# daeheepark/TrajSDE

Measured on AMD Instinct MI355X. Metric: scenes/sec (K=6, 20 SDE steps, ~256 agents) at 1/2/4/8 MI355X; minADE match, higher is better.
Workload: dtype f32 (fp16x3 split: 22-bit operands on v_mfma_f32_16x16x32_f16, f32 accumulate)

## Files before the change

### trajsde_amd/csrc/kernels.hpp

```cpp
#pragma once
#include <hip/hip_runtime.h>
#include <stdint.h>

#include "dropout.hpp"
#include "layouts.hpp"
#include "philox.hpp"

namespace tsde {

__global__ void k_aa_center(const float* img, const float* x, const float* x_fake, const float* rot, const uint8_t* bos,
                            const int32_t* orig, int N, int Nt, int H, float* center, float* cn, float* q);
template <bool X6>
__global__ void k_edge_kv(const float* img, const float* geom, const int32_t* dst, const float* q, int64_t E, float* logits, float* v,
                          int heads);
template <int THREADS>
__global__ void k_edge_kv2(const float* img, const float* geom, const int32_t* dst, const float* q, int64_t E, float* logits, float* v,
                           int heads);
constexpr int SEG_REC = 96;
constexpr int SEG_STREAMS_512 = 256 * 8 * 32;
struct AttnPlan {
  int C;
  int64_t nstreams;
  int64_t rec_slots(int64_t targets) const { return targets + nstreams + 1; }
};
// ... 93 lines not shown
    const float* _nf = nullptr;                                                                                     \
    if ((heads) == 4) {                                                                                             \
      if (_d) TS_LAUNCH_TAG("k_edge_attn_rows<4>", false, (k_global_attn<4, false, true, false>), grid, block, lds, st, img, segptr, _ns, emb, q, _nf, _nf, R, agg, stats, drop); \
      else TS_LAUNCH_TAG("k_edge_attn_rows<4>", false, (k_global_attn<4, false, false, false>), grid, block, lds, st, img, segptr, _ns, emb, q, _nf, _nf, R, agg, stats, drop); \
    } else {                                                                                                        \
      if (_d) TS_LAUNCH_TAG("k_edge_attn_rows<8>", false, (k_global_attn<8, false, true, false>), grid, block, lds, st, img, segptr, _ns, emb, q, _nf, _nf, R, agg, stats, drop); \
      else TS_LAUNCH_TAG("k_edge_attn_rows<8>", false, (k_global_attn<8, false, false, false>), grid, block, lds, st, img, segptr, _ns, emb, q, _nf, _nf, R, agg, stats, drop); \
    }                                                                                                               \
  } while (0)
__global__ void k_seg_merge(const int32_t* segptr, const float* rec, EdgeCount ec, int C, int64_t R, float* agg, float* stats, int heads,
                            const float* img, const float* q, int add_cv, int rec_layout);
template <bool DROP, bool SAVE, bool PP>
__global__ void k_edge_attn3(const float* img, const float* geom, const int32_t* dst, const float* q, EdgeCount ec, int C, float* rec, int heads,
                             const int32_t* segptr, DropArg drop, float* emb_out);
template <bool X6>
__global__ void k_edge_embed(const float* img, const float* geom, EdgeCount ec, float* emb_out, int st_bf16);
bool rel_embed_fused();
constexpr int edge_embed2_lds(int threads) { return (EdgeL6G::SIZE + (threads / 64) * ROWSTAGE) * 4; }
__global__ void k_edge_embed2(const float* img, const float* geom, EdgeCount ec, float* emb_out, int st_bf16);
template <bool X6>
__global__ void k_global_edge(const float* img, const float* rel, const int32_t* src, const int32_t* dst, const float* q,
                              const float* kn, const float* vn, int64_t E, float* logits, float* v);
template <int HEADS, bool ST_BF16, bool DROP, bool NODE>
__global__ void k_global_attn(const float* img, const int32_t* segptr, const int32_t* src, const float* rel, const float* q, const float* kn,
                              const float* vn, int64_t N, float* agg, float* stats, DropArg drop);
__global__ void k_seg_softmax_agg(const int32_t* segptr, const float* logits, const float* v, int64_t R, float* agg, int heads, DropArg drop);
template <bool X6>
__global__ void k_node_update(const float* img, const float* agg, const float* xn, const float* x, int64_t R, float* x1, float* xn2, DropArg drop,
                              SegMerge mg);
__global__ void k_ffn6(const float* img, const float* x1, const float* xn2, int64_t R, float* out, DropArg drop);
__global__ void k_ffn(const float* img, const float* x1, const float* xn2, int64_t R, float* out, DropArg drop, int out_bf16);
template <int NQ, bool SPLITKV = false>
__global__ void k_node_proj(const float* img, const float* x, int64_t R, float* xn_out, float* p0, float* p1, float* p2);
__global__ void k_mode_proj(const float* norm_g, const float* proj_g, const float* x, int64_t N, float* out);

__global__ void k_enc_sde_step(const float* img, const float* h_in, const float* hidden0, int Nt, float dt, float sq, float sn, float cs,
                               int idx, int noise_step0, NoiseArg na, const uint8_t* nus, const int32_t* eos, const int32_t* pick_slot, float* h_ode,
                               float* diff_pick);
__global__ void k_enc_gru_step(const float* img, const float* h_ode, const float* x_t, int Nt, int N, int t, int TT, int idx,
                               const uint8_t* pad, const int32_t* orig, const int32_t* eos, float* h_out, float* local_out,
                               float* latent_t);

constexpr int COOP_TMAX = 4;
constexpr int COOP_RS = 68;
constexpr int COOP_TILE = 16 * COOP_RS;
constexpr int COOP_BIAS_VECS = 21;
constexpr int coop_lds_floats(int tiles) {
  return tiles * (COOP_TILE + 5 * (TSDE_SPLIT_H3 ? 1024 : COOP_TILE)) + tiles * 64 + COOP_BIAS_VECS * 64 + 32 * 3 * 64;
}
struct StepTab {
  float dt[32], sq[32], sn[32], cs[32];
};
struct RecurTape {
  float *HIN, *H1, *H2, *G1, *G2, *GS, *HODE, *XS, *U1, *R1, *UU, *RR, *RH, *N1, *NW;
};
template <int TW, bool SAVE>
__global__ void k_enc_recur_coop(const float* sde_img, const float* gru_img, const float* coop6, const float* h0, const float* aa_out, int Nt, int N, int H,
                                 int TT, int tiles_per_wg, StepTab tab, int noise_step0, NoiseArg na, const uint8_t* nus, const uint8_t* pad,
                                 const int32_t* orig, const int32_t* eos, const int32_t* pick_slot, float* kept, float* diff_pick,
                                 float* latent_ys, int aa_bf16, RecurTape tp);
struct RecurBwdCoopArgs {
  const float *gru_t, *sde_t;
  int Nt, N, H, TT;
  NoiseArg na;
  const uint8_t *pad, *nus;
  const int32_t *orig, *eos;
// ... 43 lines not shown
```

### trajsde_amd/csrc/layouts.hpp

```cpp
#pragma once
#ifndef TSDE_SPLIT_H3
#define TSDE_SPLIT_H3 1
#endif

namespace tsde {

#define TS_FIELD(name, size, prev) name = prev##_END, name##_END = name + (size)

constexpr int MAT64 = 64 * 64;

struct AaCenterL {
  enum : int {
    S_END = 0,
    TS_FIELD(W0, 128, S), TS_FIELD(B0, 64, W0), TS_FIELD(G1, 64, B0), TS_FIELD(E1, 64, G1),
    TS_FIELD(W3, MAT64, E1), TS_FIELD(B3, 64, W3), TS_FIELD(G4, 64, B3), TS_FIELD(E4, 64, G4),
    TS_FIELD(W6, MAT64, E4), TS_FIELD(B6, 64, W6), TS_FIELD(G7, 64, B6), TS_FIELD(E7, 64, G7),
    TS_FIELD(BOS, 21 * 64, E7), TS_FIELD(N1G, 64, BOS), TS_FIELD(N1B, 64, N1G),
    TS_FIELD(WQ, MAT64, N1B), TS_FIELD(BQ, 64, WQ),
    SIZE = BQ_END
  };
};

struct EdgeL {
  enum : int {
// ... 79 lines not shown
  enum : int {
    S_END = 0,
    TS_FIELD(WIH, MAT64X6, S), TS_FIELD(BIH, 64, WIH), TS_FIELD(WHH, MAT64X6, BIH), TS_FIELD(BHH, 64, WHH),
    TS_FIELD(WSELF, MAT64X6, BHH), TS_FIELD(BSELF, 64, WSELF), TS_FIELD(WOUT, MAT64X6, BSELF), TS_FIELD(BOUT, 64, WOUT),
    TS_FIELD(N2G, 64, BOUT), TS_FIELD(N2B, 64, N2G),
    SIZE = N2B_END
  };
};
struct FfnL6 {
  enum : int {
    S_END = 0,
    TS_FIELD(W1, 2 * MAT64X6, S), TS_FIELD(B1, 128, W1), TS_FIELD(W2, 2 * MAT64X6, B1), TS_FIELD(B2, 64, W2),
    HALF = B2_END, SIZE = 2 * B2_END
  };
};
static_assert(UpdL6::SIZE * 4 <= 160 * 1024 && FfnL6::HALF * 4 <= 160 * 1024, "split-precision node images must fit LDS");

struct FfnL {
  enum : int {
    S_END = 0,
    TS_FIELD(W1, 4 * MAT64, S), TS_FIELD(B1, 256, W1), TS_FIELD(W2, 4 * MAT64, B1), TS_FIELD(B2, 64, W2),
    SIZE = B2_END
  };
};

template <int NQ>
struct NodeProjL {
  enum : int {
    S_END = 0,
    TS_FIELD(N1G, 64, S), TS_FIELD(N1B, 64, N1G), TS_FIELD(W, NQ * MAT64, N1B), TS_FIELD(B, NQ * 64, W),
    SIZE = B_END
  };
};

struct GEdgeL {
  enum : int { S_END = 0, TS_FIELD(WKV, 2 * MAT64, S), TS_FIELD(BKV, 128, WKV), SIZE = BKV_END };
};

struct DriftL {
  enum : int {
    S_END = 0,
    TS_FIELD(W0, MAT64, S), TS_FIELD(WS, 64, W0), TS_FIELD(WC, 64, WS), TS_FIELD(B0, 64, WC),
    TS_FIELD(W2, MAT64, B0), TS_FIELD(B2, 64, W2), TS_FIELD(W4, MAT64, B2), TS_FIELD(B4, 64, W4),
    SIZE = B4_END
  };
};
struct DiffL {
  enum : int {
    S_END = 0,
    TS_FIELD(W0, MAT64, S), TS_FIELD(WS, 64, W0), TS_FIELD(WC, 64, WS), TS_FIELD(B0, 64, WC),
    TS_FIELD(W2, MAT64, B0), TS_FIELD(B2, 64, W2), TS_FIELD(W4, 64, B2), TS_FIELD(B4, 4, W4),
    SIZE = B4_END
  };
};

struct DriftL6 {
  enum : int {
    S_END = 0,
    TS_FIELD(W0, MAT64X6, S), TS_FIELD(WS, 64, W0), TS_FIELD(WC, 64, WS), TS_FIELD(B0, 64, WC),
    TS_FIELD(W2, MAT64X6, B0), TS_FIELD(B2, 64, W2), TS_FIELD(W4, MAT64X6, B2), TS_FIELD(B4, 64, W4),
    SIZE = B4_END
  };
};
struct DiffL6 {
  enum : int {
    S_END = 0,
// ... 321 lines not shown
```

### trajsde_amd/csrc/stages.hip

```cpp
#include "common.hpp"
#include "kernels.hpp"
#include "layouts.hpp"

#include <algorithm>
#include <cstdlib>

namespace tsde {

static bool edge_x6() { static bool v = []() { const char* e = getenv("TRAJSDE_EDGE_FP32"); return !(e && atoi(e) != 0); }(); return v; }
static bool edge_pair() { static bool v = []() { const char* e = getenv("TRAJSDE_EDGE_PAIR"); return !(e && atoi(e) == 0); }(); return v; }
static int pair_threads() { static int t = []() { const char* e = getenv("TRAJSDE_PAIR_THREADS"); const int v = e ? atoi(e) : 768; return v == 512 ? 512 : 768; }(); return t; }
static bool attn_fused() { static bool v = []() { const char* e = getenv("TRAJSDE_ATTN_FUSED"); return !(e && atoi(e) == 0); }(); return v && edge_x6() && edge_pair() && TSDE_SPLIT_H3; }
static int fused_threads() {
  static const int t = [] { const char* e = getenv("TRAJSDE_FUSED_THREADS"); const int v = e ? atoi(e) : 512; return v == 256 ? 256 : 512; }();
  return t;
}
static bool merge_in_update() { static const bool v = []() { const char* e = getenv("TRAJSDE_MERGE_KERNEL"); return !(e && atoi(e) != 0); }(); return v; }
static bool edge_pipe() { static const bool v = []() { const char* e = getenv("TRAJSDE_EDGE_PIPE"); return e && atoi(e) == 1; }(); return v; }
static bool fused_one_tile() { static const bool v = []() { const char* e = getenv("TRAJSDE_FUSED_TILES"); return e && atoi(e) == 1; }(); return v; }
static bool edge_pingpong() { static const bool v = []() { const char* e = getenv("TRAJSDE_EDGE_PINGPONG"); return e && atoi(e) != 0; }(); return v; }
static bool edge_tile32() { static const bool v = []() { const char* e = getenv("TRAJSDE_EDGE_TILE"); return e && atoi(e) == 32; }(); return v && TSDE_SPLIT_H3; }
static bool global_fused_env() { static const bool v = []() { const char* e = getenv("TRAJSDE_GLOBAL_UNFUSED"); return !(e && atoi(e) != 0); }(); return v; }
static int fused_streams() { return 256 * 256; }
static AttnPlan fused_plan(int64_t E) { return attn_plan(E, fused_streams()); }
// ... 25 lines not shown
    hA = c.take<float>(int64_t(g->Nt) * 64); hB = c.take<float>(int64_t(g->Nt) * 64); lat = c.take<float>(N * 64);
    al_xn = c.take<float>(N * 64); al_q = c.take<float>(N * 64);
    al_logits = c.take<float>(fused ? 8 : int64_t(g->E_la) * 8 + 8); al_v = c.take<float>(fused ? 64 : int64_t(g->E_la) * 64 + 64);
    al_agg = c.take<float>(N * 64); al_x1 = c.take<float>(N * 64); al_xn2 = c.take<float>(N * 64);
    total = c.off + 256;
    ok = c.ok;
  }
};

struct AggWs {
  float *rel, *xn, *q, *kn, *vn, *logits, *v, *agg, *x1, *xn2, *xa, *xb;
  int64_t total;
  bool ok;
  AggWs(const trajsde_batch* b, const trajsde_graph* g, void* ws, int64_t bytes) {
    Carver c(ws, bytes);
    const int64_t N = b->N, E = g->E_g;
    rel = c.take<float>(E * 64 + 64);
    xn = c.take<float>(N * 64); q = c.take<float>(N * 64); kn = c.take<float>(N * 64); vn = c.take<float>(N * 64);
    logits = c.take<float>(E * 8 + 8); v = c.take<float>(E * 64 + 64);
    agg = c.take<float>(N * 64); x1 = c.take<float>(N * 64); xn2 = c.take<float>(N * 64); xa = c.take<float>(N * 64); xb = c.take<float>(N * 64);
    total = c.off + 256;
    ok = c.ok;
  }
};

static bool node_x6() {
  static bool v = []() {
    const char* e = getenv("TRAJSDE_NODE_FP32");
    return e ? atoi(e) == 0 : !TSDE_SPLIT_H3;
  }();
  return v;
}

struct NodeImgs {
  const float *upd, *ffn, *upd6, *ffn6;
};
static int update_ffn(const NodeImgs& im, const float* agg, const float* xn, const float* x, int64_t R, float* x1, float* xn2, float* out,
                      hipStream_t st, const DropArg& drop = no_drop(), bool out_bf16 = false, const SegMerge& mg = no_merge()) {
  const int64_t ntiles = (R + 15) / 16;
  TS_REQUIRE(!(out_bf16 && node_x6()), "bf16 state storage needs the one-pass FFN kernel (default fp16x3 build, TRAJSDE_NODE_FP32 unset)");
  if (node_x6()) {
    TS_LAUNCH(k_node_update<true>, tile_grid(ntiles, threads_node(), UpdL6::SIZE * 4), threads_node(), UpdL6::SIZE * 4, st, im.upd6, agg, xn, x,
              R, x1, xn2, drop, mg);
    TS_LAUNCH(k_ffn6, tile_grid(ntiles, threads_node(), FfnL6::HALF * 4), threads_node(), FfnL6::HALF * 4, st, im.ffn6, x1, xn2, R, out, drop);
  } else {
    TS_LAUNCH(k_node_update<false>, tile_grid(ntiles, threads_node(), UpdL::SIZE * 4), threads_node(), UpdL::SIZE * 4, st, im.upd, agg, xn, x, R,
              x1, xn2, drop, mg);
    TS_LAUNCH(k_ffn, tile_grid(ntiles, threads_node(), FfnL::SIZE * 4), threads_node(), FfnL::SIZE * 4, st, im.ffn, x1, xn2, R, out, drop, out_bf16 ? 1 : 0);
  }
  return TRAJSDE_OK;
}
static int attention_tail(const NodeImgs& im, const int32_t* segptr, const float* logits, const float* v, const float* xn, const float* x,
                          int64_t R, float* agg, float* x1, float* xn2, float* out, hipStream_t st, int heads = 8,
                          const DropArg& drop = no_drop()) {
  TS_LAUNCH(k_seg_softmax_agg, cdiv(R, 4), 256, 0, st, segptr, logits, v, R, agg, heads, drop);
  return update_ffn(im, agg, xn, x, R, x1, xn2, out, st, drop);
}

int fused_edge_attention(const char* tag, bool dominant, const float* img, const float* geom, const int32_t* dst, const float* q,
                         const EdgeCount& ec, const int32_t* segptr, int64_t R, float* rec, float* agg, int heads, hipStream_t st,
                         const DropArg& drop, float* emb_out, float* stats, SegMerge* defer) {
  const int64_t E = ec.E;
  const AttnPlan pl = fused_plan(E);
  TS_REQUIRE(E < (int64_t(1) << 28), "fused edge attention: an edge list of 2^28 or more entries exceeds its 32-bit byte offsets; split the batch");
  if (E > 0) {
    const int threads = fused_threads();
    const int64_t streams = ec.dev ? std::min<int64_t>(E, fused_streams()) : pl.nstreams;
    const int per_wg = (fused_one_tile() ? 1024 : threads) / 64 * (fused_one_tile() ? 16 : 32);
    const int grid = xcd_grid((streams + per_wg - 1) / per_wg);
    const int lds = (EdgeL6F::LDS_SIZE + 256 * 64) * 4;
    const bool d = drop.p > 0.f, sv = emb_out != nullptr;
#define TS_EA2H(N_, D_, S_, L_, H_) TS_LAUNCH_TAG(tag, dominant, (k_edge_attn2<N_, D_, S_, L_, H_>), grid, threads, lds, st, img, geom, dst, q, ec, pl.C, rec, heads, segptr, drop, emb_out)
#define TS_EA2L(N_, D_, S_, L_) do { if (heads == 8) TS_EA2H(N_, D_, S_, L_, true); else TS_EA2H(N_, D_, S_, L_, false); } while (0)
// ... 337 lines not shown
static int aggregator_forward_impl(const trajsde_batch* b, const trajsde_graph* g, const float* blob, int num_layers, int num_modes,
                                   int num_heads, const float* local_embed, void* ws, int64_t ws_bytes, float* global_embed,
                                   const trajsde_dropout* dropout, void* stream_, bool rel_ready);

int trajsde_aggregator_forward_heads(const trajsde_batch* b, const trajsde_graph* g, const float* blob, int num_layers, int num_modes,
                                     int num_heads, const float* local_embed, void* ws, int64_t ws_bytes, float* global_embed,
                                     const trajsde_dropout* dropout, void* stream_) {
  return aggregator_forward_impl(b, g, blob, num_layers, num_modes, num_heads, local_embed, ws, ws_bytes, global_embed, dropout, stream_, false);
}

int trajsde_aggregator_forward_prepared(const trajsde_batch* b, const trajsde_graph* g, const float* blob, int num_layers, int num_modes,
                                        int num_heads, const float* local_embed, void* ws, int64_t ws_bytes, float* global_embed,
                                        const trajsde_dropout* dropout, void* stream_) {
  return aggregator_forward_impl(b, g, blob, num_layers, num_modes, num_heads, local_embed, ws, ws_bytes, global_embed, dropout, stream_, true);
}

static int aggregator_forward_impl(const trajsde_batch* b, const trajsde_graph* g, const float* blob, int num_layers, int num_modes,
                                   int num_heads, const float* local_embed, void* ws, int64_t ws_bytes, float* global_embed,
                                   const trajsde_dropout* dropout, void* stream_, bool rel_ready) {
  TS_REQUIRE(b && g && blob && local_embed && ws && global_embed, "aggregator_forward: null pointer");
  TS_REQUIRE(!dropout || (dropout->p >= 0.f && dropout->p < 1.f), "aggregator_forward: dropout p must be in [0, 1)");
  TS_REQUIRE(num_heads == 8 || num_heads == 4, "aggregator_forward: num_heads must be 8 or 4");
  TS_REQUIRE(g->g_src && g->g_segptr, "aggregator_forward: graph not compacted (call trajsde_graph_compact)");
  TS_REQUIRE(num_layers >= 0 && num_modes > 0, "aggregator_forward: bad layer/mode count");
  AggWs w(b, g, ws, ws_bytes);
  if (!w.ok) return fail(TRAJSDE_ERR_WORKSPACE, "aggregator_forward: workspace too small");
  hipStream_t st = static_cast<hipStream_t>(stream_);
  const int64_t N = b->N, E = g->E_g, ntiles = (N + 15) / 16, etiles = (E + 15) / 16;
  const bool split = rel_split_possible() && num_heads == 8 && (!dropout || dropout->p == 0.f) && E > 0;
  if (!rel_ready || split != rel_split_possible())
    if (int rc = aggregator_rel_embed(b, g, blob, w, st, split)) return rc;
  const float* x = local_embed;
  float* bufs[2] = {w.xa, w.xb};
  for (int i = 0; i < num_layers; ++i) {
    const float* lb = blob + AggBlob::layer(i);
    if (split)
      TS_LAUNCH((k_node_proj<3, true>), tile_grid(ntiles, 512, NodeProjL<3>::SIZE * 4), 512, NodeProjL<3>::SIZE * 4, st, lb + AggLayerL::QKV, x, N,
                w.xn, w.q, w.kn, w.vn);
    else
      TS_LAUNCH(k_node_proj<3>, tile_grid(ntiles, 512, NodeProjL<3>::SIZE * 4), 512, NodeProjL<3>::SIZE * 4, st, lb + AggLayerL::QKV, x, N,
                w.xn, w.q, w.kn, w.vn);
    float* out = bufs[i & 1];
    const NodeImgs im{lb + AggLayerL::UPD, lb + AggLayerL::FFN, lb + AggLayerL::UPD6, lb + AggLayerL::FFN6};
    const bool fused = global_fused_env() || num_heads != 8;
    const DropArg drop = dropout ? make_drop(dropout->p, dropout->seed, 2 + i) : no_drop();
    TS_REQUIRE(fused || drop.p == 0.f, "aggregator_forward: dropout needs the fused global attention (unset TRAJSDE_GLOBAL_UNFUSED)");
    TS_REQUIRE(fused || !state_bf16(), "aggregator_forward: bf16 state storage needs the fused global attention");
    TS_REQUIRE(fused || g->exact, "aggregator_forward: a graph from trajsde_graph_prepare_async needs the fused global attention");
    if (fused) {
      TS_REQUIRE(N < (1 << 23), "aggregator_forward: node rows are addressed with 32-bit byte offsets (N < 2^23)");
      if (split && rel_split_scene_cache() && b->batch != nullptr && b->A > 0 && b->A + 2 <= E * 8 + 8) {
        int32_t* scene_ptr = reinterpret_cast<int32_t*>(w.logits);
        if (i == 0)
          if (int rc = launch_scene_ptr(b->batch, b->N, b->A, g->g_src, g->g_dst, g->g_segptr, E, scene_ptr, st)) return rc;
        if (int rc = launch_global_attn_sc(lb + AggLayerL::ATTN, g->g_segptr, g->g_src, w.rel, w.q, w.kn, w.vn, N, b->A, b->batch, scene_ptr, w.agg, st))
          return rc;
      } else if (split) {
        if (int rc = launch_global_attn_h3(lb + AggLayerL::ATTN, g->g_segptr, g->g_src, w.rel, w.q, w.kn, w.vn, N, w.agg, st)) return rc;
      } else if (num_heads == 8 && !state_bf16() && drop.p == 0.f && gattn_mm_enabled()) {
        if (int rc = launch_global_attn_mm(lb + AggLayerL::ATTN, g->g_segptr, g->g_src, w.rel, w.q, w.kn, w.vn, N, w.agg, st)) return rc;
      } else if (num_heads == 8 && !state_bf16() && gattn_f32mm_enabled() && E > 0) {
        if (int rc = launch_global_attn_mf(lb + AggLayerL::ATTN, g->g_segptr, g->g_src, w.rel, w.q, w.kn, w.vn, N, w.agg, nullptr, drop, st)) return rc;
      } else {
        TS_GLOBAL_ATTN(num_heads, state_bf16(), drop, xcd_grid(cdiv(N, 4)), 256, 0, st, lb + AggLayerL::ATTN, g->g_segptr, g->g_src, w.rel, w.q, w.kn, w.vn, N, w.agg, static_cast<float*>(nullptr));
      }
      if (int rc = update_ffn(im, w.agg, w.xn, x, N, w.x1, w.xn2, out, st, drop)) return rc;
      x = out;
      continue;
    }
    if (E > 0) {
      if (edge_x6())
        TS_LAUNCH(k_global_edge<true>, tile_grid(etiles, 512, GEdgeL6::SIZE * 4), 512, GEdgeL6::SIZE * 4, st,
                  lb + AggLayerL::EDGE6, w.rel, g->g_src, g->g_dst, w.q, w.kn, w.vn, E, w.logits, w.v);
      else
        TS_LAUNCH(k_global_edge<false>, tile_grid(etiles, 512, GEdgeL::SIZE * 4), 512, GEdgeL::SIZE * 4, st,
                  lb + AggLayerL::EDGE, w.rel, g->g_src, g->g_dst, w.q, w.kn, w.vn, E, w.logits, w.v);
    }
    if (int rc = attention_tail(im, g->g_segptr, w.logits, w.v, w.xn, x, N, w.agg, w.x1, w.xn2, out, st)) return rc;
    x = out;
  }
  const int lds = (128 + MAT64 + 64) * 4;
  dim3 grid(tile_grid(ntiles, 512, lds), num_modes);
  TS_LAUNCH(k_mode_proj, grid, 512, lds, st, blob + AggBlob::norm(num_layers), blob + AggBlob::proj(num_layers, 0), x, N, global_embed);
  return TRAJSDE_OK;
}

}
```

### trajsde_amd/csrc/prep.hip

```cpp

#include <algorithm>
#include <cmath>
#include <limits>
#include <atomic>
#include <cstdlib>
#include <cstring>

#include "common.hpp"
#include "philox.hpp"
#include "tile.hpp"

namespace tsde {

__global__ void k_rotate(const float* __restrict__ ang, int N, const float* __restrict__ y, int F,
                         float* __restrict__ rot, float* __restrict__ y_rot) {
  const int per = F > 0 && y != nullptr ? F : 1;
  const int64_t idx = int64_t(blockIdx.x) * blockDim.x + threadIdx.x;
  if (idx >= int64_t(N) * per) return;
  const int i = int(idx / per), t = int(idx - int64_t(i) * per);
  const float s = sinf(ang[i]), c = cosf(ang[i]);
  if (t == 0) {
    f4 r = {c, -s, s, c};
    *reinterpret_cast<f4*>(rot + 4 * i) = r;
  }
// ... 2 lines not shown
    y_rot[(int64_t(i) * F + t) * 2] = a * c + b * s;
    y_rot[(int64_t(i) * F + t) * 2 + 1] = b * c - a * s;
  }
}


constexpr int DONE_WAYS = 16;
__device__ __forceinline__ bool last_block_done(unsigned int* counters , unsigned int total) {
  __shared__ int s_last;
  asm volatile("s_waitcnt vmcnt(0)" ::: "memory");
  __syncthreads();
  if (threadIdx.x == 0) {
    const unsigned way = blockIdx.x % DONE_WAYS;
    const unsigned quota = total / DONE_WAYS + (way < total % DONE_WAYS ? 1u : 0u);
    int last = 0;
    if (__hip_atomic_fetch_add(&counters[way], 1u, __ATOMIC_RELAXED, __HIP_MEMORY_SCOPE_AGENT) + 1u == quota) {
      unsigned ways_used = total < unsigned(DONE_WAYS) ? total : unsigned(DONE_WAYS);
      last = __hip_atomic_fetch_add(&counters[DONE_WAYS], 1u, __ATOMIC_RELAXED, __HIP_MEMORY_SCOPE_AGENT) + 1u == ways_used;
    }
    s_last = last;
  }
  __syncthreads();
  return s_last != 0;
}
struct CoherentI32 {
  __amdgpu_buffer_rsrc_t rs;
  __device__ __forceinline__ explicit CoherentI32(const int32_t* base)
      : rs(__builtin_amdgcn_make_buffer_rsrc(const_cast<int32_t*>(base), 0, 0xFFFFFFFF, 0x00020000)) {}
  __device__ __forceinline__ int32_t operator[](int i) const { return __builtin_amdgcn_raw_buffer_load_b32(rs, i * 4, 0, 16 ); }
};
__device__ __forceinline__ void store_through(int32_t* p, int32_t v) { __hip_atomic_store(p, v, __ATOMIC_RELAXED, __HIP_MEMORY_SCOPE_AGENT); }

constexpr int EPT = 16;
__device__ __forceinline__ void degree_body(int blk, const int64_t* __restrict__ ei, int E, int32_t* __restrict__ deg) {
  int d[EPT];
#pragma unroll
  for (int u = 0; u < EPT; ++u) {
    const int e = (blk * EPT + u) * 256 + int(threadIdx.x);
    d[u] = e < E ? int(ei[int64_t(E) + e]) : -1;
  }
#pragma unroll
  for (int u = 0; u < EPT; ++u)
    if (d[u] >= 0) atomicAdd(&deg[d[u]], 1);
}
__device__ __forceinline__ void scatter_body(int blk, const int64_t* __restrict__ ei, int E, const int32_t* __restrict__ rowptr,
                                             int32_t* __restrict__ deg, int32_t* __restrict__ out) {
  int d[EPT], p[EPT], src[EPT];
#pragma unroll
  for (int u = 0; u < EPT; ++u) {
    const int e = (blk * EPT + u) * 256 + int(threadIdx.x);
    d[u] = e < E ? int(ei[int64_t(E) + e]) : -1;
    src[u] = e < E ? int32_t(ei[e]) : 0;
  }
#pragma unroll
  for (int u = 0; u < EPT; ++u) p[u] = d[u] >= 0 ? rowptr[d[u]] + atomicSub(&deg[d[u]], 1) - 1 : -1;
#pragma unroll
  for (int u = 0; u < EPT; ++u)
    if (p[u] >= 0) out[p[u]] = src[u];
}
__device__ __forceinline__ void scatter_lane_body(int blk, const int64_t* __restrict__ lai, int E, const int32_t* __restrict__ rowptr,
                                                  int32_t* __restrict__ deg, int64_t* __restrict__ out) {
  int d[EPT], p[EPT];
  int64_t key[EPT];
#pragma unroll
  for (int u = 0; u < EPT; ++u) {
    const int e = (blk * EPT + u) * 256 + int(threadIdx.x);
    d[u] = e < E ? int(lai[int64_t(E) + e]) : -1;
    key[u] = e < E ? ((lai[e] << 32) | int64_t(e)) : 0;
  }
#pragma unroll
  for (int u = 0; u < EPT; ++u) p[u] = d[u] >= 0 ? rowptr[d[u]] + atomicSub(&deg[d[u]], 1) - 1 : -1;
#pragma unroll
  for (int u = 0; u < EPT; ++u)
    if (p[u] >= 0) out[p[u]] = key[u];
}
__global__ __launch_bounds__(256) void k_scatter2(const int64_t* __restrict__ ei, int E, const int32_t* __restrict__ rowptr, int32_t* __restrict__ deg,
                                                  int32_t* __restrict__ csr_src, int nb_a, const int64_t* __restrict__ lai, int Ea,
                                                  const int32_t* __restrict__ la_rowptr, int32_t* __restrict__ la_deg, int64_t* __restrict__ la_pack) {
  const int blk = blockIdx.x;
  if (blk < nb_a) scatter_body(blk, ei, E, rowptr, deg, csr_src);
  else scatter_lane_body(blk - nb_a, lai, Ea, la_rowptr, la_deg, la_pack);
}
template <typename T, typename EMIT>
__device__ __forceinline__ void sort_long_rows(int vblk, int vgrid, const int32_t* __restrict__ rowptr, int n_rows, T* __restrict__ vals,
                                               T* buf , int32_t* __restrict__ low_out, int32_t* __restrict__ row_out,
                                               const EMIT& emit) {
  const T INF = sizeof(T) == 8 ? T(INT64_MAX) : T(INT32_MAX);
  for (int row = vblk; row < n_rows; row += vgrid) {
    const int beg = rowptr[row], n = rowptr[row + 1] - beg;
    if (n <= 256) continue;
    if (row_out != nullptr)
      for (int i = threadIdx.x; i < n; i += blockDim.x) row_out[beg + i] = row;
    int P = 2;
    while (P < n) P <<= 1;
    if (P <= 4096) {
      for (int i = threadIdx.x; i < P; i += blockDim.x) buf[i] = i < n ? vals[beg + i] : INF;
      __syncthreads();
      for (int k = 2; k <= P; k <<= 1)
        for (int j = k >> 1; j > 0; j >>= 1) {
          for (int i = threadIdx.x; i < P; i += blockDim.x) {
            const int l = i ^ j;
            if (l > i) {
              const T vi = buf[i], vl = buf[l];
              const bool up = (i & k) == 0;
              if ((vi > vl) == up) {
                buf[i] = vl;
                buf[l] = vi;
              }
            }
          }
          __syncthreads();
        }
      for (int i = threadIdx.x; i < n; i += blockDim.x) {
        vals[beg + i] = buf[i];
// ... 239 lines not shown
    }
    int32_t inc[2] = {sum[0], sum[1]};
#pragma unroll
    for (int d = 1; d < 64; d <<= 1) {
      const int32_t o0 = __shfl_up(inc[0], d), o1 = __shfl_up(inc[1], d);
      if (lane >= d) { inc[0] += o0; inc[1] += o1; }
    }
    if (lane == 63) { s_w[0][wv] = inc[0]; s_w[1][wv] = inc[1]; }
    __syncthreads();
#pragma unroll
    for (int a = 0; a < 2; ++a) {
      int32_t run = s_carry[a] + inc[a] - sum[a];
      for (int w = 0; w < wv; ++w) run += s_w[a][w];
      int32_t* out = a ? out1 : out0;
#pragma unroll
      for (int c = 0; c < PT; ++c) {
        const int i = base + PT * t + c;
        if (i < n) out[i] = run;
        run += v[a][c];
      }
    }
    __syncthreads();
    if (t < 2) s_carry[t] += s_w[t][0] + s_w[t][1] + s_w[t][2] + s_w[t][3];
    __syncthreads();
  }
}

struct FirstPassArgs {
  int N, A, H, TT, L, P, E, Ea, b0, b1, b2, b3, b4, b5, blocks;
  const int64_t *edge_index, *lane_actor_index, *agent_index, *batch, *source;
  const uint8_t *bos, *pad;
  const float *x, *pos, *lane_pos, *lane_pad;
  int32_t *deg, *la_deg, *rowptr, *la_rowptr, *orig, *eos, *pick_slot;
  uint8_t* nus;
  float *x_fake, *lane_feat;
  float2 *pos_t, *x_t;
  uint32_t* vmask;
  unsigned int* done;
  NoiseArg na;
};
__global__ __launch_bounds__(256) void k_prep_first(const FirstPassArgs a) {
  const int blk = blockIdx.x, i = threadIdx.x;
  if (blk < a.b0) degree_body(blk, a.edge_index, a.E, a.deg);
  else if (blk < a.b1) degree_body(blk - a.b0, a.lane_actor_index, a.Ea, a.la_deg);
  else if (blk < a.b2) ext_nodes_body((blk - a.b1) * 256 + i, a.N, a.A, a.H, a.agent_index, a.batch, a.source, a.bos, a.orig, a.nus, a.eos, a.pick_slot);
  else if (blk < a.b3) fake_x_body((blk - a.b2) * 256 + i, a.A, a.H, a.x, a.agent_index, a.na, a.x_fake);
  else if (blk < a.b4) valid_mask_body((blk - a.b3) * 256 + i, a.N, a.H, a.TT, a.pad, a.vmask);
  else if (blk < a.b5) time_major_body(blk - a.b4, a.N, a.H, a.TT, a.pos, a.x, a.pos_t, a.x_t);
  else lane_feat_body((blk - a.b5) * 256 + i, a.L, a.P, a.lane_pos, a.lane_pad, a.lane_feat);
  if (!last_block_done(a.done, unsigned(a.blocks))) return;
  block_scan_two(a.deg, a.rowptr, a.la_deg, a.la_rowptr, a.N + 1);
}

__global__ __launch_bounds__(256) void k_row_sort2(int N, int nb_a, int nb_l, const int32_t* __restrict__ rowptr, int32_t* __restrict__ csr_src,
                                                   int32_t* __restrict__ csr_dst, const uint32_t* __restrict__ vmask, int tref, int E,
                                                   uint8_t* __restrict__ flags_g, const int32_t* __restrict__ la_rowptr,
                                                   int64_t* __restrict__ la_pack, int32_t* __restrict__ la_eid, int32_t* __restrict__ la_actor,
                                                   const float* __restrict__ vec, float radius, int Ea, uint8_t* __restrict__ flags_la) {
  __shared__ int64_t buf[4096];
  const int blk = blockIdx.x;
  if (blk == 0 && threadIdx.x == 0) {
    flags_g[E] = 0;
    flags_la[Ea] = 0;
  }
  if (blk < nb_a) {
    if (E <= 0) return;
    auto emit = [&](int p, int32_t sender, int row) { flags_g[p] = uint8_t((vmask[sender] >> tref) & (vmask[row] >> tref) & 1u); };
    row_sort_part<int32_t>(blk, nb_a, rowptr, N, csr_src, nullptr, csr_dst, reinterpret_cast<int32_t*>(buf), emit);
  } else {
    if (Ea <= 0) return;
    auto emit = [&](int p, int64_t packed, int row) {
      (void)row;
      const int64_t e = packed & 0xFFFFFFFFll;
      flags_la[p] = uint8_t(sqrtf(norm2_sq(vec[2 * e], vec[2 * e + 1])) < radius);
    };
    row_sort_part<int64_t>(blk - nb_a, nb_l, la_rowptr, N, la_pack, la_eid, la_actor, buf, emit);
  }
// ... 447 lines not shown
  return w.total;
}

static int graph_prepare(const trajsde_batch* b, const float* rot, float radius, const trajsde_noise* fake_noise, void* ws,
                         int64_t ws_bytes, trajsde_graph* out, void* stream_, bool sync) {
  if (int rc = check_batch(b)) return rc;
  TS_REQUIRE(rot && ws && out, "graph_prepare: null pointer");
  PrepWs w(b, ws, ws_bytes);
  if (!w.ok) return fail(TRAJSDE_ERR_WORKSPACE, "graph_prepare: workspace too small");
  hipStream_t st = static_cast<hipStream_t>(stream_);
  const int N = b->N, A = b->A, E = b->E, H = b->H, TT = b->TT, Ea = b->E_al, Nt = N + A;
  NoiseArg na{0, nullptr, nullptr};
  if (fake_noise) { na.seed = fake_noise->seed; na.z = fake_noise->z; na.row_ids = fake_noise->row_ids; na.seed_dev = fake_noise->seed_dev; }

  TS_HIP(hipMemsetAsync(w.deg, 0, size_t(w.zeroed_bytes), st));
  const int tref = H - 1;
  {
    ProfScope ps("k_prep_first", st);
    FirstPassArgs fa;
    fa.N = N; fa.A = A; fa.H = H; fa.TT = TT; fa.L = b->L; fa.P = b->lane_pts; fa.E = E; fa.Ea = Ea;
    fa.b0 = cdiv(E, 256 * EPT);
    fa.b1 = fa.b0 + cdiv(Ea, 256 * EPT);
    fa.b2 = fa.b1 + cdiv(Nt, 256);
    fa.b3 = fa.b2 + (A > 0 ? cdiv(A * ((2 * H + 3) / 4), 256) : 0);
    fa.b4 = fa.b3 + cdiv(N, 256);
    fa.b5 = fa.b4 + cdiv(int64_t(N) * H, 1024);
    fa.blocks = fa.b5 + (b->L > 0 ? cdiv(b->L, 256) : 0);
    fa.edge_index = b->edge_index; fa.lane_actor_index = b->lane_actor_index; fa.agent_index = b->agent_index; fa.batch = b->batch;
    fa.source = b->source; fa.bos = b->bos_mask; fa.pad = b->padding_mask; fa.x = b->x; fa.pos = b->positions;
    fa.lane_pos = b->lane_positions; fa.lane_pad = b->lane_paddings;
    fa.deg = w.deg; fa.la_deg = w.la_deg; fa.rowptr = w.rowptr; fa.la_rowptr = w.la_rowptr; fa.orig = w.orig; fa.eos = w.eos;
    fa.pick_slot = w.pick_slot; fa.nus = w.nus; fa.x_fake = w.x_fake; fa.lane_feat = w.lane_feat; fa.pos_t = w.pos_t; fa.x_t = w.x_t;
    fa.vmask = w.vmask; fa.done = w.done + 0; fa.na = na;
    k_prep_first<<<fa.blocks, 256, 0, st>>>(fa);
  }
  if (E > 0 || Ea > 0) {
    ProfScope ps("k_scatter2", st);
    const int nb_a = cdiv(E, 256 * EPT);
    k_scatter2<<<nb_a + cdiv(Ea, 256 * EPT), 256, 0, st>>>(b->edge_index, E, w.rowptr, w.deg, w.csr_src, nb_a, b->lane_actor_index, Ea, w.la_rowptr,
                                                     w.la_deg, w.la_pack);
  }
  {
    ProfScope ps("k_row_sort2", st);
    const int per_list = cdiv(N, 4) < 8192 ? cdiv(N, 4) : 8192;
    k_row_sort2<<<2 * per_list, 256, 0, st>>>(N, per_list, per_list, w.rowptr, w.csr_src, w.csr_dst, w.vmask, tref, E, w.flags_g, w.la_rowptr,
                                              w.la_pack, w.la_eid, w.la_actor, b->lane_actor_vectors, radius, Ea, w.flags_la);
  }
  {
    ProfScope ps("k_aa_count", st);
    const AaArgs aa = aa_args(b, w, rot, radius);
    k_aa_count<<<int(w.aa_blocks), 256, 0, st>>>(aa);
  }
  {
    ProfScope ps("k_scan_multi", st);
    ScanMultiArgs sa;
    std::memset(&sa, 0, sizeof(sa));
    int64_t nmax = 0;
    auto add = [&](const void* in, int32_t* out_, int64_t n, int u8, int inst) {
      ScanJob& j = sa.j[sa.njobs++];
      j.in = in; j.out = out_; j.n = int(n); j.u8 = u8; j.st = w.scan_st + int64_t(inst) * SCAN_WORDS;
      nmax = std::max(nmax, n);
    };
    add(w.aa_segptr, w.aa_segptr, w.n_aa + 1, 0, 0);
    add(w.flags_g, w.cpos_g, int64_t(E) + 1, 1, 1);
    add(w.flags_la, w.cpos_la, int64_t(Ea) + 1, 1, 2);
    TS_REQUIRE(nmax <= int64_t(SCAN_MAX_BLOCKS) * 65536, "graph stage: more than 33 M elements in a prefix sum");
    const int64_t per = (nmax + int64_t(SCAN_MAX_BLOCKS) * 1024 - 1) / (int64_t(SCAN_MAX_BLOCKS) * 1024);
    const int PER = per <= 8 ? 8 : (per <= 16 ? 16 : (per <= 32 ? 32 : 64));
    for (int q = 0; q < sa.njobs; ++q) {
      sa.j[q].blocks = cdiv(sa.j[q].n, PER * 1024);
      sa.blocks += sa.j[q].blocks;
    }
    if (PER == 8) k_scan_multi<8><<<sa.blocks, 1024, 0, st>>>(sa);
// ... 85 lines not shown
```

Before: 16130.

## Fuse node update, FFN and next-layer QKV projection into one kernel

Adds k_node_block, which runs the gated node update, both FFN linears, and optionally the next layer's layernorm and QKV projection in a single launch. It stages the weight images in two phases, reusing the same LDS region. This removes intermediate x1/xn2 global round trips and one or two kernel launches per aggregator layer. In exchange, each block restages weights per round with extra barriers. By default it is only used when all tiles fit in one round, and it writes xn into the buffer that is also read as input.

Result: no change. 16200, median of 6 (+0.4%).

```diff
diff --git a/trajsde_amd/csrc/kernels.hpp b/trajsde_amd/csrc/kernels.hpp
--- a/trajsde_amd/csrc/kernels.hpp
+++ b/trajsde_amd/csrc/kernels.hpp
@@ -149,6 +149,9 @@
 __global__ void k_ffn(const float* img, const float* x1, const float* xn2, int64_t R, float* out, DropArg drop, int out_bf16);
 template <int NQ, bool SPLITKV = false>
 __global__ void k_node_proj(const float* img, const float* x, int64_t R, float* xn_out, float* p0, float* p1, float* p2);
+template <bool PROJ>
+__global__ void k_node_block(const float* upd, const float* ffn, const float* proj, const float* agg, const float* xn, const float* x,
+                             int64_t R, float* out, SegMerge mg, float* xn_next, float* p0, float* p1, float* p2);
 __global__ void k_mode_proj(const float* norm_g, const float* proj_g, const float* x, int64_t N, float* out);
 
 __global__ void k_enc_sde_step(const float* img, const float* h_in, const float* hidden0, int Nt, float dt, float sq, float sn, float cs,
diff --git a/trajsde_amd/csrc/layouts.hpp b/trajsde_amd/csrc/layouts.hpp
--- a/trajsde_amd/csrc/layouts.hpp
+++ b/trajsde_amd/csrc/layouts.hpp
@@ -135,6 +135,16 @@
     SIZE = B_END
   };
 };
+
+struct NodeBlockL {
+  enum : int {
+    S_END = 0,
+    TS_FIELD(A, UpdL::SIZE, S), TS_FIELD(B, 4 * MAT64 + 256, A), TS_FIELD(B2, 64, B),
+    SIZE = B2_END
+  };
+};
+static_assert(FfnL::B1 == FfnL::W1 + 4 * MAT64 && 4 * MAT64 <= UpdL::SIZE && NodeProjL<3>::SIZE <= 4 * MAT64 + 256 &&
+              NodeBlockL::SIZE * 4 <= 160 * 1024, "k_node_block: the second images are staged over the first");
 
 struct GEdgeL {
   enum : int { S_END = 0, TS_FIELD(WKV, 2 * MAT64, S), TS_FIELD(BKV, 128, WKV), SIZE = BKV_END };
diff --git a/trajsde_amd/csrc/node_block.hip b/trajsde_amd/csrc/node_block.hip
--- /dev/null
+++ b/trajsde_amd/csrc/node_block.hip
@@ -0,0 +1,147 @@
+#include "common.hpp"
+#include "kernels.hpp"
+#include "layouts.hpp"
+#include "range.hpp"
+#include "tile.hpp"
+
+namespace tsde {
+
+#if TSDE_SPLIT_H3
+template <bool PROJ>
+__global__ __launch_bounds__(512) void k_node_block(const float* __restrict__ upd_g, const float* __restrict__ ffn_g,
+                                                    const float* __restrict__ proj_g, const float* __restrict__ agg, const float* xn,
+                                                    const float* __restrict__ x, int64_t R, float* __restrict__ out, SegMerge mg,
+                                                    float* xn_next, float* __restrict__ p0, float* __restrict__ p1,
+                                                    float* __restrict__ p2) {
+  extern __shared__ __attribute__((aligned(16))) float lds[];
+  using U = UpdL;
+  using P = NodeProjL<3>;
+  float* const lds_a = lds + NodeBlockL::A;
+  float* const lds_b = lds + NodeBlockL::B;
+  const float* const b2 = lds + NodeBlockL::B2;
+  const Lane L;
+  const int waves = blockDim.x >> 6, wave = __builtin_amdgcn_readfirstlane(int(threadIdx.x >> 6));
+  const int64_t ntiles = (R + 15) / 16;
+  stage_copy(lds + NodeBlockL::B2, ffn_g + FfnL::B2, 64);
+  const int64_t first = int64_t(blockIdx.x) * waves, stride = int64_t(gridDim.x) * waves;
+  for (int64_t base = first; base < ntiles; base += stride) {
+    if (base != first) __syncthreads();
+    stage_copy(lds_a, upd_g, U::SIZE);
+    stage_copy(lds_b, ffn_g + FfnL::W1, NodeBlockL::B_END - NodeBlockL::B);
+    __syncthreads();
+    keep_lds_reads_here();
+    const int64_t tile = base + wave;
+    const bool live = tile < ntiles;
+    const int64_t row = tile * 16 + L.n, r = row < R ? row : R - 1;
+    f4 x1[4], hid[16];
+    if (live) {
+      f4 a[4], n[4], g[4], s[4];
+      if (mg.rec != nullptr) {
+        const int C = stream_len(mg.ec, edge_count(mg.ec), mg.C_host);
+        const int beg = mg.segptr[r], end = mg.segptr[r + 1];
+#pragma unroll
+        for (int jt = 0; jt < 4; ++jt) a[jt] = f4{0.f, 0.f, 0.f, 0.f};
+        if (end > beg) {
+          const StreamMap smap = stream_map(C);
+          const int c0 = int(stream_of(smap, beg)), c1 = int(stream_of(smap, end - 1));
+          const float* rr = mg.rec + (r + c0) * SEG_REC;
+#pragma unroll
+          for (int jt = 0; jt < 4; ++jt) a[jt] = *reinterpret_cast<const f4*>(rr + 16 * jt + 4 * L.g);
+          f4 m = *reinterpret_cast<const f4*>(rr + 64 + 4 * L.g), sm = *reinterpret_cast<const f4*>(rr + 80 + 4 * L.g);
+          for (int c = c0 + 1; c <= c1; ++c) {
+            rr += SEG_REC;
+            const f4 mp = *reinterpret_cast<const f4*>(rr + 64 + 4 * L.g), sp = *reinterpret_cast<const f4*>(rr + 80 + 4 * L.g);
+#pragma unroll
+            for (int jt = 0; jt < 4; ++jt) {
+              const f4 ap = *reinterpret_cast<const f4*>(rr + 16 * jt + 4 * L.g);
+              const float mn = fmaxf(m[jt], mp[jt]);
+              const float wa = fast_exp(m[jt] - mn), wb = fast_exp(mp[jt] - mn);
+              sm[jt] = sm[jt] * wa + sp[jt] * wb;
+              a[jt] = a[jt] * wa + ap * wb;
+              m[jt] = mn;
+            }
+          }
+#pragma unroll
+          for (int jt = 0; jt < 4; ++jt) {
+            const f4 cv = *reinterpret_cast<const f4*>(mg.cv + 16 * jt + 4 * L.g);
+#pragma unroll
+            for (int c = 0; c < 4; ++c) a[jt][c] = a[jt][c] / (sm[jt] + 1e-16f) + cv[c];
+          }
+        }
+      } else {
+        load_row(a, agg, r, L.g);
+      }
+      load_row(n, xn, r, L.g);
+      f4 xr[4];
+      load_row(xr, x, r, L.g);
+      range_note(absmax<4>(a), RS_NODE_AGG);
+      linear<4, 4>(g, a, lds_a + U::WIH, lds_a + U::BIH, L);
+      {
+        f4 h[4];
+        linear<4, 4>(h, n, lds_a + U::WHH, lds_a + U::BHH, L);
+#pragma unroll
+        for (int jt = 0; jt < 4; ++jt) g[jt] += h[jt];
+      }
+      sigmoid_<4>(g);
+      linear<4, 4>(s, n, lds_a + U::WSELF, lds_a + U::BSELF, L);
+#pragma unroll
+      for (int jt = 0; jt < 4; ++jt)
+#pragma unroll
+        for (int c = 0; c < 4; ++c) a[jt][c] = a[jt][c] + g[jt][c] * (s[jt][c] - a[jt][c]);
+      range_note(absmax<4>(a), RS_NODE_AGG);
+      linear<4, 4>(s, a, lds_a + U::WOUT, lds_a + U::BOUT, L);
+#pragma unroll
+      for (int jt = 0; jt < 4; ++jt) x1[jt] = n[jt] = xr[jt] + s[jt];
+      layer_norm<4>(n, lds_a + U::N2G, lds_a + U::N2B, L.g);
+      linear<16, 4>(hid, n, lds_b, lds_b + 4 * MAT64, L);
+      relu<16>(hid);
+      range_note(absmax<16>(hid), RS_FFN_HIDDEN);
+    }
+    __syncthreads();
+    stage_copy(lds_a, ffn_g + FfnL::W2, 4 * MAT64);
+    if (PROJ) stage_copy(lds_b, proj_g, P::SIZE);
+    __syncthreads();
+    keep_lds_reads_here();
+    if (live) {
+      f4 o[4];
+      linear<4, 16>(o, hid, lds_a, b2, L);
+#pragma unroll
+      for (int jt = 0; jt < 4; ++jt) o[jt] += x1[jt];
+      if (row < R) store_row(o, out, row, L.g);
+      if (PROJ) {
+        f4 pr[12];
+        layer_norm<4>(o, lds_b + P::N1G, lds_b + P::N1B, L.g);
+        if (row < R) store_row(o, xn_next, row, L.g);
+        linear<12, 4>(pr, o, lds_b + P::W, lds_b + P::B, L);
+        float* outs[3] = {p0, p1, p2};
+#pragma unroll
+        for (int j = 0; j < 3; ++j) {
+          f4 t4[4] = {pr[4 * j], pr[4 * j + 1], pr[4 * j + 2], pr[4 * j + 3]};
+          if (j > 0) {
+            if (row < R) {
+              char* o8 = reinterpret_cast<char*>(outs[j] + row * 64);
+#pragma unroll
+              for (int jt = 0; jt < 4; ++jt) {
+                unsigned h0, l0, h1, l1;
+                split_pair(t4[jt][0], t4[jt][1], h0, l0);
+                split_pair(t4[jt][2], t4[jt][3], h1, l1);
+                *reinterpret_cast<uint2*>(o8 + 32 * jt + 8 * L.g) = uint2{h0, h1};
+                *reinterpret_cast<uint2*>(o8 + 128 + 32 * jt + 8 * L.g) = uint2{l0, l1};
+              }
+            }
+            continue;
+          }
+          if (row < R) store_row(t4, outs[j], row, L.g);
+        }
+      }
+    }
+  }
+}
+
+template __global__ void k_node_block<false>(const float*, const float*, const float*, const float*, const float*, const float*, int64_t, float*,
+                                             SegMerge, float*, float*, float*, float*);
+template __global__ void k_node_block<true>(const float*, const float*, const float*, const float*, const float*, const float*, int64_t, float*,
+                                            SegMerge, float*, float*, float*, float*);
+#endif
+
+}
diff --git a/trajsde_amd/csrc/stages.hip b/trajsde_amd/csrc/stages.hip
--- a/trajsde_amd/csrc/stages.hip
+++ b/trajsde_amd/csrc/stages.hip
@@ -81,13 +81,43 @@
   return v;
 }
 
+static int node_fuse() { static const int v = []() { const char* e = getenv("TRAJSDE_NODE_FUSE"); return e ? atoi(e) : 1; }(); return v; }
+constexpr int64_t NODE_BLOCK_ONE_ROUND = 256 * 8;
+static bool node_block_serves(int64_t R, const DropArg& drop, bool out_bf16) {
+#if TSDE_SPLIT_H3
+  static const bool plain = getenv("TRAJSDE_NODE_FP32") == nullptr && threads_node() == 512;
+  return plain && node_fuse() != 0 && drop.p == 0.f && !out_bf16 && R > 0 && (node_fuse() == 2 || (R + 15) / 16 <= NODE_BLOCK_ONE_ROUND);
+#else
+  (void)R; (void)drop; (void)out_bf16;
+  return false;
+#endif
+}
+
 struct NodeImgs {
   const float *upd, *ffn, *upd6, *ffn6;
 };
+struct NextProj {
+  const float* img;
+  float *xn, *q, *kn, *vn;
+};
 static int update_ffn(const NodeImgs& im, const float* agg, const float* xn, const float* x, int64_t R, float* x1, float* xn2, float* out,
-                      hipStream_t st, const DropArg& drop = no_drop(), bool out_bf16 = false, const SegMerge& mg = no_merge()) {
+                      hipStream_t st, const DropArg& drop = no_drop(), bool out_bf16 = false, const SegMerge& mg = no_merge(),
+                      const NextProj* next = nullptr) {
   const int64_t ntiles = (R + 15) / 16;
   TS_REQUIRE(!(out_bf16 && node_x6()), "bf16 state storage needs the one-pass FFN kernel (default fp16x3 build, TRAJSDE_NODE_FP32 unset)");
+#if TSDE_SPLIT_H3
+  if (node_block_serves(R, drop, out_bf16)) {
+    const int grid = tile_grid(ntiles, 512, NodeBlockL::SIZE * 4);
+    if (next)
+      TS_LAUNCH((k_node_block<true>), grid, 512, NodeBlockL::SIZE * 4, st, im.upd, im.ffn, next->img, agg, xn, x, R, out, mg, next->xn, next->q,
+                next->kn, next->vn);
+    else
+      TS_LAUNCH((k_node_block<false>), grid, 512, NodeBlockL::SIZE * 4, st, im.upd, im.ffn, static_cast<const float*>(nullptr), agg, xn, x, R, out,
+                mg, static_cast<float*>(nullptr), static_cast<float*>(nullptr), static_cast<float*>(nullptr), static_cast<float*>(nullptr));
+    return TRAJSDE_OK;
+  }
+#endif
+  TS_REQUIRE(next == nullptr, "update_ffn: the next layer's projection rides on the fused launch only");
   if (node_x6()) {
     TS_LAUNCH(k_node_update<true>, tile_grid(ntiles, threads_node(), UpdL6::SIZE * 4), threads_node(), UpdL6::SIZE * 4, st, im.upd6, agg, xn, x,
               R, x1, xn2, drop, mg);
@@ -491,9 +521,12 @@
     if (int rc = aggregator_rel_embed(b, g, blob, w, st, split)) return rc;
   const float* x = local_embed;
   float* bufs[2] = {w.xa, w.xb};
+  bool proj_done = false;
   for (int i = 0; i < num_layers; ++i) {
     const float* lb = blob + AggBlob::layer(i);
-    if (split)
+    if (proj_done)
+      proj_done = false;
+    else if (split)
       TS_LAUNCH((k_node_proj<3, true>), tile_grid(ntiles, 512, NodeProjL<3>::SIZE * 4), 512, NodeProjL<3>::SIZE * 4, st, lb + AggLayerL::QKV, x, N,
                 w.xn, w.q, w.kn, w.vn);
     else
@@ -523,7 +556,9 @@
       } else {
         TS_GLOBAL_ATTN(num_heads, state_bf16(), drop, xcd_grid(cdiv(N, 4)), 256, 0, st, lb + AggLayerL::ATTN, g->g_segptr, g->g_src, w.rel, w.q, w.kn, w.vn, N, w.agg, static_cast<float*>(nullptr));
       }
-      if (int rc = update_ffn(im, w.agg, w.xn, x, N, w.x1, w.xn2, out, st, drop)) return rc;
+      const NextProj next{blob + AggBlob::layer(i + 1) + AggLayerL::QKV, w.xn, w.q, w.kn, w.vn};
+      proj_done = split && i + 1 < num_layers && node_block_serves(N, drop, false);
+      if (int rc = update_ffn(im, w.agg, w.xn, x, N, w.x1, w.xn2, out, st, drop, false, no_merge(), proj_done ? &next : nullptr)) return rc;
       x = out;
       continue;
     }
```

## Rank edges per block in shared-memory hash table to cut global atomics in CSR build

Applied to the files above, without the earlier changes.

The degree-counting pass now groups each block's edges by destination in a shared-memory open-addressing hash table. It issues one global atomicAdd per distinct destination instead of one per edge, and records each edge's position within its row. The scatter pass reads these precomputed in-row positions instead of doing a global atomicSub per edge. This trades contended global atomics for shared-memory CAS work, an extra int32 write and read per edge, and LDS use in every k_prep_first block. It falls back to per-edge atomics when probing overflows, and it reuses the cpos_g/cpos_la buffers as scratch, which assumes those are free and large enough at this stage.

After: 16270 before, 16250 after, median of 2. No clear change (-0.1%).

```diff
diff --git a/trajsde_amd/csrc/prep.hip b/trajsde_amd/csrc/prep.hip
--- a/trajsde_amd/csrc/prep.hip
+++ b/trajsde_amd/csrc/prep.hip
@@ -58,34 +58,94 @@
 __device__ __forceinline__ void store_through(int32_t* p, int32_t v) { __hip_atomic_store(p, v, __ATOMIC_RELAXED, __HIP_MEMORY_SCOPE_AGENT); }
 
 constexpr int EPT = 16;
-__device__ __forceinline__ void degree_body(int blk, const int64_t* __restrict__ ei, int E, int32_t* __restrict__ deg) {
-  int d[EPT];
+constexpr int RANK_SLOTS = 1024, RANK_PROBES = 8;
+struct RankTable {
+  int32_t key[RANK_SLOTS];
+  int32_t cnt[RANK_SLOTS];
+  int overflow;
+};
+__device__ __forceinline__ bool block_rank(const int (&d)[EPT], int (&slot)[EPT], int (&r)[EPT], RankTable& s) {
+  const int tid = int(threadIdx.x);
+  for (int i = tid; i < RANK_SLOTS; i += 256) {
+    s.key[i] = -1;
+    s.cnt[i] = 0;
+  }
+  if (tid == 0) s.overflow = 0;
+  __syncthreads();
 #pragma unroll
   for (int u = 0; u < EPT; ++u) {
-    const int e = (blk * EPT + u) * 256 + int(threadIdx.x);
+    slot[u] = -1;
+    r[u] = 0;
+    if (d[u] < 0) continue;
+    int h = d[u] & (RANK_SLOTS - 1);
+    for (int probe = 0; probe < RANK_PROBES; ++probe) {
+      const int k = atomicCAS(&s.key[h], -1, d[u]);
+      if (k == -1 || k == d[u]) {
+        slot[u] = h;
+        break;
+      }
+      h = (h + 1) & (RANK_SLOTS - 1);
+    }
+    if (slot[u] >= 0) r[u] = atomicAdd(&s.cnt[slot[u]], 1);
+    else s.overflow = 1;
+  }
+  __syncthreads();
+  return s.overflow == 0;
+}
+__device__ __forceinline__ void degree_body(int blk, const int64_t* __restrict__ ei, int E, int32_t* __restrict__ deg,
+                                            int32_t* __restrict__ inrow, RankTable& s) {
+  const int tid = int(threadIdx.x);
+  int d[EPT], slot[EPT], r[EPT];
+#pragma unroll
+  for (int u = 0; u < EPT; ++u) {
+    const int e = (blk * EPT + u) * 256 + tid;
     d[u] = e < E ? int(ei[int64_t(E) + e]) : -1;
   }
+  if (!block_rank(d, slot, r, s)) {
+#pragma unroll
+    for (int u = 0; u < EPT; ++u) r[u] = d[u] >= 0 ? atomicAdd(&deg[d[u]], 1) : 0;
+#pragma unroll
+    for (int u = 0; u < EPT; ++u)
+      if (d[u] >= 0) inrow[(blk * EPT + u) * 256 + tid] = r[u];
+    return;
+  }
+  {
+    constexpr int SPT = RANK_SLOTS / 256;
+    int c[SPT], k[SPT];
+#pragma unroll
+    for (int q = 0; q < SPT; ++q) {
+      c[q] = s.cnt[q * 256 + tid];
+      k[q] = s.key[q * 256 + tid];
+    }
+#pragma unroll
+    for (int q = 0; q < SPT; ++q)
+      if (c[q] > 0) c[q] = atomicAdd(&deg[k[q]], c[q]);
+#pragma unroll
+    for (int q = 0; q < SPT; ++q) s.cnt[q * 256 + tid] = c[q];
+  }
+  __syncthreads();
 #pragma unroll
   for (int u = 0; u < EPT; ++u)
-    if (d[u] >= 0) atomicAdd(&deg[d[u]], 1);
+    if (d[u] >= 0) inrow[(blk * EPT + u) * 256 + tid] = s.cnt[slot[u]] + r[u];
 }
 __device__ __forceinline__ void scatter_body(int blk, const int64_t* __restrict__ ei, int E, const int32_t* __restrict__ rowptr,
-                                             int32_t* __restrict__ deg, int32_t* __restrict__ out) {
+                                             const int32_t* __restrict__ inrow, int32_t* __restrict__ out) {
   int d[EPT], p[EPT], src[EPT];
 #pragma unroll
   for (int u = 0; u < EPT; ++u) {
     const int e = (blk * EPT + u) * 256 + int(threadIdx.x);
     d[u] = e < E ? int(ei[int64_t(E) + e]) : -1;
     src[u] = e < E ? int32_t(ei[e]) : 0;
-  }
-#pragma unroll
-  for (int u = 0; u < EPT; ++u) p[u] = d[u] >= 0 ? rowptr[d[u]] + atomicSub(&deg[d[u]], 1) - 1 : -1;
+    p[u] = e < E ? inrow[e] : 0;
+  }
+#pragma unroll
+  for (int u = 0; u < EPT; ++u) p[u] = d[u] >= 0 ? rowptr[d[u]] + p[u] : -1;
 #pragma unroll
   for (int u = 0; u < EPT; ++u)
     if (p[u] >= 0) out[p[u]] = src[u];
 }
 __device__ __forceinline__ void scatter_lane_body(int blk, const int64_t* __restrict__ lai, int E, const int32_t* __restrict__ rowptr,
-                                                  int32_t* __restrict__ deg, int64_t* __restrict__ out) {
+                                                  const int32_t* __restrict__ inrow, int64_t* __restrict__ out) {
   int d[EPT], p[EPT];
   int64_t key[EPT];
 #pragma unroll
@@ -93,19 +153,20 @@
     const int e = (blk * EPT + u) * 256 + int(threadIdx.x);
     d[u] = e < E ? int(lai[int64_t(E) + e]) : -1;
     key[u] = e < E ? ((lai[e] << 32) | int64_t(e)) : 0;
-  }
-#pragma unroll
-  for (int u = 0; u < EPT; ++u) p[u] = d[u] >= 0 ? rowptr[d[u]] + atomicSub(&deg[d[u]], 1) - 1 : -1;
+    p[u] = e < E ? inrow[e] : 0;
+  }
+#pragma unroll
+  for (int u = 0; u < EPT; ++u) p[u] = d[u] >= 0 ? rowptr[d[u]] + p[u] : -1;
 #pragma unroll
   for (int u = 0; u < EPT; ++u)
     if (p[u] >= 0) out[p[u]] = key[u];
 }
-__global__ __launch_bounds__(256) void k_scatter2(const int64_t* __restrict__ ei, int E, const int32_t* __restrict__ rowptr, int32_t* __restrict__ deg,
+__global__ __launch_bounds__(256) void k_scatter2(const int64_t* __restrict__ ei, int E, const int32_t* __restrict__ rowptr, const int32_t* __restrict__ inrow,
                                                   int32_t* __restrict__ csr_src, int nb_a, const int64_t* __restrict__ lai, int Ea,
-                                                  const int32_t* __restrict__ la_rowptr, int32_t* __restrict__ la_deg, int64_t* __restrict__ la_pack) {
+                                                  const int32_t* __restrict__ la_rowptr, const int32_t* __restrict__ la_inrow, int64_t* __restrict__ la_pack) {
   const int blk = blockIdx.x;
-  if (blk < nb_a) scatter_body(blk, ei, E, rowptr, deg, csr_src);
-  else scatter_lane_body(blk - nb_a, lai, Ea, la_rowptr, la_deg, la_pack);
+  if (blk < nb_a) scatter_body(blk, ei, E, rowptr, inrow, csr_src);
+  else scatter_lane_body(blk - nb_a, lai, Ea, la_rowptr, la_inrow, la_pack);
 }
 template <typename T, typename EMIT>
 __device__ __forceinline__ void sort_long_rows(int vblk, int vgrid, const int32_t* __restrict__ rowptr, int n_rows, T* __restrict__ vals,
@@ -411,6 +472,7 @@
   const uint8_t *bos, *pad;
   const float *x, *pos, *lane_pos, *lane_pad;
   int32_t *deg, *la_deg, *rowptr, *la_rowptr, *orig, *eos, *pick_slot;
+  int32_t *inrow, *la_inrow;
   uint8_t* nus;
   float *x_fake, *lane_feat;
   float2 *pos_t, *x_t;
@@ -419,9 +481,10 @@
   NoiseArg na;
 };
 __global__ __launch_bounds__(256) void k_prep_first(const FirstPassArgs a) {
+  __shared__ RankTable s_rank;
   const int blk = blockIdx.x, i = threadIdx.x;
-  if (blk < a.b0) degree_body(blk, a.edge_index, a.E, a.deg);
-  else if (blk < a.b1) degree_body(blk - a.b0, a.lane_actor_index, a.Ea, a.la_deg);
+  if (blk < a.b0) degree_body(blk, a.edge_index, a.E, a.deg, a.inrow, s_rank);
+  else if (blk < a.b1) degree_body(blk - a.b0, a.lane_actor_index, a.Ea, a.la_deg, a.la_inrow, s_rank);
   else if (blk < a.b2) ext_nodes_body((blk - a.b1) * 256 + i, a.N, a.A, a.H, a.agent_index, a.batch, a.source, a.bos, a.orig, a.nus, a.eos, a.pick_slot);
   else if (blk < a.b3) fake_x_body((blk - a.b2) * 256 + i, a.A, a.H, a.x, a.agent_index, a.na, a.x_fake);
   else if (blk < a.b4) valid_mask_body((blk - a.b3) * 256 + i, a.N, a.H, a.TT, a.pad, a.vmask);
@@ -935,13 +998,14 @@
     fa.deg = w.deg; fa.la_deg = w.la_deg; fa.rowptr = w.rowptr; fa.la_rowptr = w.la_rowptr; fa.orig = w.orig; fa.eos = w.eos;
     fa.pick_slot = w.pick_slot; fa.nus = w.nus; fa.x_fake = w.x_fake; fa.lane_feat = w.lane_feat; fa.pos_t = w.pos_t; fa.x_t = w.x_t;
     fa.vmask = w.vmask; fa.done = w.done + 0; fa.na = na;
+    fa.inrow = w.cpos_g; fa.la_inrow = w.cpos_la;
     k_prep_first<<<fa.blocks, 256, 0, st>>>(fa);
   }
   if (E > 0 || Ea > 0) {
     ProfScope ps("k_scatter2", st);
     const int nb_a = cdiv(E, 256 * EPT);
-    k_scatter2<<<nb_a + cdiv(Ea, 256 * EPT), 256, 0, st>>>(b->edge_index, E, w.rowptr, w.deg, w.csr_src, nb_a, b->lane_actor_index, Ea, w.la_rowptr,
-                                                     w.la_deg, w.la_pack);
+    k_scatter2<<<nb_a + cdiv(Ea, 256 * EPT), 256, 0, st>>>(b->edge_index, E, w.rowptr, w.cpos_g, w.csr_src, nb_a, b->lane_actor_index, Ea,
+                                                           w.la_rowptr, w.cpos_la, w.la_pack);
   }
   {
     ProfScope ps("k_row_sort2", st);
```
